# ReactiveBayes/RxInfer.jl

Measured on AMD Instinct MI355X. Metric: node-message-updates/sec (d=4 LGSSM, T=100k, BP sweep with Bethe free energy), higher is better.
Workload: dtype f64; 1 GPU; LGSSM d=4 dy=4 T=100000, 1024 independent chains per GPU (BASELINE config 2), 1 BP sweep + Bethe free energy per step; chain c drawn from numpy default_rng(42+c); chains_per_gpu=1024, T=100000, segments=128, segment_len=782

## Files before the change

### rxinfer.jl_amd/csrc/launch_tables.hpp

```cpp
#pragma once
#include <hip/hip_runtime.h>

#include <cstdlib>

#include "lgssm_kernels.hpp"
#include "predict_kernels.hpp"
#include "noise_kernels.hpp"
#ifndef RXHIP_LAUNCH_LGSSM_ONLY
#include "dense_kernels.hpp"
#include "dense_tab_kernels.hpp"
#include "dense_mseg_kernels.hpp"
#include "dense_split_kernels.hpp"
#include "dense8_kernels.hpp"
#endif

#ifndef RXHIP_TAB_SAME_TOL
#define RXHIP_TAB_SAME_TOL 5e-15
#endif

namespace rxhip {

struct SweepArgs {
    bool rev;
    int bnd;
    bool write_cov;
    int y_ring;
    int waves;
};
struct LgssmVtbl {
    int d, dy;
    int cst_size, tab_size, agg_size;
    int oA, oP, oLOBS, oG, oQI, oC0, oM1, oV1, oHF;
    int tK, tU;
    int aPI, aC, aJ, aCI, aX, aJJ;
    int scan_size, sM1, sM2, sVB, sN1, sN2, sLB;
    int f0_size, fK, fU, fSI, pos_size, pPI, pJ, pC, fs_size, fsA1, fsA2, fsW, mt_row;
    void (*forward0)(const Params&, const double*, bool, bool, int, hipStream_t);
    void (*time_tables)(const TimeTabParams&, hipStream_t);
    void (*fe_seg)(const Params&, hipStream_t);
    int gt_row, se_size;
    void (*smooth_tables)(const SmoothTabParams&, const double*, hipStream_t);
    void (*backward_sh)(const Params&, const double*, const double* gtab, const double* segend, const SweepArgs&, hipStream_t);
    void (*boundary_scan_tab)(const Params&, const double*, bool, hipStream_t);
    void (*seg_aggregate)(const Params&, const double*, bool, hipStream_t);
    int ex_size;
    void (*seg_elements)(const Params&, hipStream_t);
    void (*boundary_scan)(const Params&, const double*, bool, bool, hipStream_t);
    void (*forward)(const Params&, const double*, bool, bool, hipStream_t);
    void (*backward)(const Params&, const double*, bool, hipStream_t);
    void (*forecast)(const PredictParams&, hipStream_t);
    void (*predict)(const PredictParams&, hipStream_t);
    void (*joint)(const PredictParams&, hipStream_t);
    void (*stream_step)(const StreamParams&, hipStream_t);
    void (*small_sweep)(const Params&, const double*, bool, hipStream_t);
    int noise_prior_size;
    void (*noise_reset)(const NoiseParams&, hipStream_t);
    void (*noise_update)(const NoiseParams&, hipStream_t);
};
void lgssm_vtbls_d1(LgssmVtbl* out);
void lgssm_vtbls_d2(LgssmVtbl* out);
void lgssm_vtbls_d3(LgssmVtbl* out);
void lgssm_vtbls_d4(LgssmVtbl* out);

inline unsigned nblk(long long n, int b) { return (unsigned)((n + b - 1) / b); }

inline const char* hook_env(const char* name) {
    const char* on = std::getenv("RXHIP_TEST_HOOKS");
    return (on && on[0] == '1' && on[1] == 0) ? std::getenv(name) : nullptr;
}

#ifndef RXHIP_LAUNCH_LGSSM_ONLY
constexpr int FE_RESID_MAX_PASSES = 8;
struct DenseVtbl {
    int nt;
    hipError_t (*prepare)();
    void (*prepare_bnd)(const DenseParams&, hipStream_t);
    void (*seg_aggregate)(const DenseParams&, hipStream_t);
    void (*boundary_scan)(const DenseParams&, bool fe, hipStream_t);
    void (*forward)(const DenseParams&, bool fe, hipStream_t);
    void (*forward_info)(const DenseParams&, bool fe, hipStream_t, long long chains);
    void (*backward_info)(const DenseParams&, bool fe, hipStream_t, long long chains);
    void (*fe_resid)(const DenseParams&, hipStream_t, int passes);
    hipError_t (*tab_prepare)();
    hipError_t (*tab_build)(const TabParams&, hipStream_t);
    void (*tab_consts)(const TabParams&, unsigned models, size_t lds, hipStream_t);
    hipError_t (*mseg_prepare)();
    void (*mseg_sweep)(const MsegParams&, const DenseParams&, bool fe, bool filter, hipStream_t);
    void (*mseg_filter_out)(const MsegParams&, const DenseParams&, hipStream_t);
    hipError_t (*split_prepare)();
    void (*split_forward)(const SplitParams&, dim3 grid, hipStream_t);
    void (*split_backward)(const SplitParams&, dim3 grid, hipStream_t);
    void (*cross_from_records)(const DenseParams&, double* cross, dim3 grid, hipStream_t);
};
const DenseVtbl* dense_vtbl_nt1();
const DenseVtbl* dense_vtbl_nt2();
const DenseVtbl* dense_vtbl_nt3();
const DenseVtbl* dense_vtbl_nt4();
#endif

}
```

### rxinfer.jl_amd/csrc/lgssm_kernels.hpp

```cpp
#pragma once
#include <hip/hip_runtime.h>
#include <stdint.h>

namespace rxhip {

constexpr int ST_NOT_POSDEF = 1;
constexpr int ST_NONFINITE = 2;
__device__ __forceinline__ void lds_barrier() {
    __builtin_amdgcn_fence(__ATOMIC_RELEASE, "workgroup", "local");
    __builtin_amdgcn_s_barrier();
    __builtin_amdgcn_fence(__ATOMIC_ACQUIRE, "workgroup", "local");
}
__device__ __forceinline__ bool is_finite(double x) { return (__double2hiint(x) & 0x7ff00000) != 0x7ff00000; }

#ifndef RXHIP_NT_STORES
#define RXHIP_NT_STORES 0
#endif
typedef double rx_d2v __attribute__((ext_vector_type(2)));
__device__ __forceinline__ void stream_store(double2* p, double a, double b) {
#if RXHIP_NT_STORES
    rx_d2v v = {a, b};
    __builtin_nontemporal_store(v, reinterpret_cast<rx_d2v*>(p));
#else
    *p = make_double2(a, b);
#endif
}

__device__ __forceinline__ void lds_put(double2& dst, const rx_d2v v) { dst = make_double2(v.x, v.y); }
template <class T>
__device__ __forceinline__ void lds_put(T& dst, const T& v) { dst = v; }
template <int NPIECES, int W, class T = rx_d2v>
struct LdsStream {
    static constexpr int TPB = 64 * W;
    static constexpr int PPL = (NPIECES + TPB - 1) / TPB;
    const int tid;
    T tr[PPL];
    __device__ __forceinline__ explicit LdsStream(const int tid_) : tid(tid_) {}
    template <class Piece>
    __device__ __forceinline__ void fetch(Piece&& piece) {
#pragma unroll
        for (int k = 0; k < PPL; ++k) piece(k * TPB + tid, tr[k]);
    }
    template <class B>
    __device__ __forceinline__ void stash(B* buf) const {
#pragma unroll
        for (int k = 0; k < PPL; ++k) {
            const int idx = k * TPB + tid;
            if ((k + 1) * TPB <= NPIECES || idx < NPIECES) lds_put(buf[idx], tr[k]);
        }
    }
    static __device__ __forceinline__ void publish() {
        if constexpr (W == 1) {
            __builtin_amdgcn_fence(__ATOMIC_RELEASE, "wavefront");
            __builtin_amdgcn_wave_barrier();
        } else {
            __builtin_amdgcn_fence(__ATOMIC_RELEASE, "workgroup", "local");
            __builtin_amdgcn_s_barrier();
            __builtin_amdgcn_fence(__ATOMIC_ACQUIRE, "workgroup", "local");
        }
    }
    template <class B>
    __device__ __forceinline__ void flip(B* buf, const bool store = true) {
        __builtin_amdgcn_fence(__ATOMIC_ACQUIRE, "wavefront");
        __builtin_amdgcn_wave_barrier();
        if (store) stash(buf);
        publish();
    }
};

template <int D>
struct Dim {
    static constexpr int NS = D * (D + 1) / 2;
    static constexpr int NP = D + NS;
    static constexpr int NP2 = (NP + 1) / 2;
};

__host__ __device__ constexpr int sidx(int i, int j) { return i >= j ? i * (i + 1) / 2 + j : j * (j + 1) / 2 + i; }

template <int D>
struct Sym {
    double v[D * (D + 1) / 2];
    __device__ __forceinline__ double& operator()(int i, int j) { return v[sidx(i, j)]; }
    __device__ __forceinline__ const double& operator()(int i, int j) const { return v[sidx(i, j)]; }
};

// ... 1141 lines not shown
    }
    if (live) f0_epilogue<D, FE>(p, seg, chain, m, eta, q0);
}

template <int D, int DY, bool FE, int W>
__global__ void __launch_bounds__(64 * W) k_forward0_ck(Params p, const CstArg<CstLayout<D, DY>::SIZE> cb) {
    using FL = F0Layout<D, DY>;
    using FS = F0Stage<D, DY>;
    constexpr int MT = TimeTab<D>::MT;
    constexpr int U = FS::U, NPF = FS::NPF, NPC = FS::NPC;
    __shared__ double2 tbuf[2][NPC];
    const int wv = W > 1 ? __builtin_amdgcn_readfirstlane((int)(threadIdx.x >> 6)) : 0;
    const int lane = W > 1 ? (int)(threadIdx.x & 63) : (int)threadIdx.x;
    const long long g0 = ((long long)blockIdx.x * W + wv) * 64;
    const long long seg = g0 / p.n_chains;
    const long long chain = g0 - seg * p.n_chains + lane;
    const long long len = seg_len(p, seg);
    const CPtr c{cb.v};
    const long long t0 = seg * p.L + 1;
    const int lg = p.ck_log2;
    const long long kmask = (1LL << lg) - 1;
    const long long f_last = p.L * (FL::SIZE / 2) - 1;
    const long long m_last = p.T * (MT / 2) - 1;
    const rx_d2v* f2 = reinterpret_cast<const rx_d2v*>(p.ftab);
    const rx_d2v* m2 = reinterpret_cast<const rx_d2v*>(p.mtab);

    double m[D], eta[D], q0 = 0.0;
#pragma unroll
    for (int i = 0; i < D; ++i) m[i] = eta[i] = 0.0;
    if (len > 0) {
        LdsStream<NPC, W> ts(threadIdx.x);
        ts.fetch([](const int, rx_d2v& v) { v = rx_d2v{0.0, 0.0}; });
        auto has_ck = [&](long long i0) { return ((i0 + U) >> lg) != (i0 >> lg) || (i0 < len && len <= i0 + U); };
        auto chunk = [&](long long i0) {
            return [&, i0, ck = has_ck(i0)](int idx, rx_d2v& v) {
                idx = idx < NPC ? idx : NPC - 1;
                if (idx < NPF) {
                    const long long gi = i0 * (FL::SIZE / 2) + idx;
                    v = f2[gi < f_last ? gi : f_last];
                } else if (ck) {
                    const long long gi = (t0 + i0) * (MT / 2) + (idx - NPF);
                    v = m2[gi < m_last ? gi : m_last];
                }
            };
        };
        ts.fetch(chunk(0));
        ts.stash(tbuf[0]);
        ts.publish();

        double yb[U][DY], yn[U][DY];
        auto y_index = [&](long long i) { return t0 + (i < len ? i : len - 1); };
#pragma unroll
        for (int u = 0; u < U; ++u) load_y<DY>(p.y, y_index(u), p.n_chains, chain, yn[u]);
        auto step = [&](const int u, const long long i, const int b) __attribute__((always_inline)) {
            const double* tb = reinterpret_cast<const double*>(&tbuf[b][0]) + u * FL::SIZE;
            const double* mt = reinterpret_cast<const double*>(&tbuf[b][NPF]) + u * MT;
            f0_step<D, DY, FE>(c, tb, yb[u], m, eta, q0);
            if (((i + 1) & kmask) != 0 && i + 1 != len) return;
            f0_store_z<D>(p, 1 + seg * p.nck + (i >> lg), chain, m, eta, mt);
        };
        int b = 0;
        long long i0 = 0;
        for (; i0 + U <= len; i0 += U, b ^= 1) {
            ts.fetch(chunk(i0 + U));
#pragma unroll
            for (int u = 0; u < U; ++u) {
#pragma unroll
                for (int k = 0; k < DY; ++k) yb[u][k] = yn[u][k];
                load_y<DY>(p.y, y_index(i0 + U + u), p.n_chains, chain, yn[u]);
            }
#pragma unroll
            for (int u = 0; u < U; ++u) step(u, i0 + u, b);
            ts.flip(tbuf[b ^ 1]);
        }
#pragma unroll
        for (int u = 0; u < U; ++u)
#pragma unroll
            for (int k = 0; k < DY; ++k) yb[u][k] = yn[u][k];
#pragma unroll
        for (int u = 0; u < U - 1; ++u)
            if (i0 + u < len) step(u, i0 + u, b);
    }
    f0_epilogue<D, FE>(p, seg, chain, m, eta, q0);
}

struct TimeTabParams {
    long long T, L;
    const double* pos;
    const double* scan;
    double* mtab;
    double* ntab;
    double* vtab;
    int* status;
};
template <int D>
__global__ void __launch_bounds__(64) k_time_tables(TimeTabParams q) {
    using PL = PosLayout<D>;
    using SL = ScanLayout<D>;
    constexpr int NS = Dim<D>::NS;
    constexpr int MT = TimeTab<D>::MT;
    const long long t = (long long)blockIdx.x * blockDim.x + threadIdx.x;
    if (t >= q.T) return;
    if (t == 0) {
#pragma unroll
        for (int k = 0; k < NS; ++k) q.vtab[k] = q.scan[SL::VB + k];
#pragma unroll
        for (int k = 0; k < MT; ++k) q.mtab[k] = q.ntab[k] = 0.0;
        return;
    }
    const long long s = (t - 1) / q.L, i = t - s * q.L;
    const double* ps = q.pos + (i - 1) * PL::SIZE;
    const double* sc = q.scan + s * SL::SIZE;
    Sym<D> Vs, Vi, T1, W;
    double det;
    bool ok = true;
#pragma unroll
    for (int k = 0; k < NS; ++k) Vs.v[k] = sc[SL::VB + k];
    ok = spd_inv<D>(Vs, Vi, det) && ok;
#pragma unroll
    for (int k = 0; k < NS; ++k) T1.v[k] = Vi.v[k] + ps[PL::J + k];
    ok = spd_inv<D>(T1, W, det) && ok;
    double M[D][D], N[D][D];
#pragma unroll
    for (int a = 0; a < D; ++a)
#pragma unroll
        for (int b = 0; b < D; ++b) {
            double acc = 0.0;
#pragma unroll
            for (int k = 0; k < D; ++k) acc += ps[PL::PI + a * D + k] * W(k, b);
            M[a][b] = acc;
        }
#pragma unroll
    for (int a = 0; a < D; ++a)
#pragma unroll
        for (int b = 0; b < D; ++b) {
            double acc = 0.0;
#pragma unroll
            for (int k = 0; k < D; ++k) acc += M[a][k] * Vi(k, b);
            N[a][b] = acc;
        }
    double* mo = q.mtab + t * MT;
    double* no = q.ntab + t * MT;
#pragma unroll
    for (int a = 0; a < D; ++a)
#pragma unroll
        for (int b = 0; b < D; ++b) {
            mo[a * D + b] = M[a][b];
            no[a * D + b] = N[a][b];
        }
    if (D * D < MT) mo[MT - 1] = no[MT - 1] = 0.0;
    double* vo = q.vtab + t * NS;
#pragma unroll
    for (int a = 0; a < D; ++a)
#pragma unroll
        for (int b = 0; b <= a; ++b) {
            double acc = ps[PL::C + sidx(a, b)];
#pragma unroll
            for (int k = 0; k < D; ++k) acc += M[a][k] * ps[PL::PI + b * D + k];
            vo[sidx(a, b)] = acc;
        }
    if (!ok) atomicOr(q.status, ST_NOT_POSDEF);
}

template <int D>
__global__ void __launch_bounds__(64) k_fe_seg(Params p) {
    using FS = FeSegLayout<D>;
// ... 2106 lines not shown
```

### rxinfer.jl_amd/csrc/lgssm_plan.hpp

```cpp
#pragma once
#include <algorithm>
#include <cmath>
#include <cstdlib>
#include <cstring>
#include <string>

namespace rxhip {
namespace plan {

#define RXHIP_SCHEDULE_HOOKS(X)                                                                                                        \
    X(int, one_pass, -1)                                                                          \
    X(bool, one_segment, false)                                                                                  \
    X(bool, backward_lanes, false)                                                                            \
    X(bool, mean_records, false)                                                                              \
    X(int, mean_checkpoint, 0)                    \
    X(Text, mean_checkpoint_text, Text{})                                                   \
    X(bool, boundary_kernel, false)                                                                        \
    X(bool, small_sweep_off, false)                                                                            \
    X(bool, elem_full, false)                                                                                      \
    X(bool, noise_moments_pass, false)                                                                    \
    X(bool, no_pack, false)                                                                                          \
    X(int, dense_split, -1)                                      \
    X(bool, host_tables, false)                                                                                  \
    X(bool, gseq, false)                                                                                                \
    X(bool, stepm_gseq, false)                                                                                    \
    X(bool, filter_gseq, false)                                                                                  \
    X(bool, joints_gseq, false)                                                                                  \
    X(int, mseg_scan, 0)                                                 \
    X(bool, mseg_one_level, false)                                                                            \
    X(int, mseg_group, 0)                                                                          \
    X(unsigned long long, mseg_max_bytes, ~0ULL)                                         \
    X(bool, wave8_off, false)                                                                                        \
    X(bool, no_frozen, false)                                                                                      \
    X(bool, cov_every_sweep, false)                                                                        \
    X(int, y_ring, 0)                                      \
    X(int, sweep_waves, 0)

struct Text { char s[16] = {0}; };

struct ScheduleHooks {
#define X(type, field, dflt) type field = dflt;
    RXHIP_SCHEDULE_HOOKS(X)
#undef X
    template <class Get>
    static ScheduleHooks read(Get get) {
        ScheduleHooks h;
        auto set = [&](const char* n) { return get(n) != nullptr; };
        auto is0 = [&](const char* n) { const char* v = get(n); return v && std::atoi(v) == 0; };
        auto not0 = [&](const char* n) { const char* v = get(n); return v && std::atoi(v) != 0; };
        auto tri = [&](const char* n) { const char* v = get(n); return v ? (std::atoi(v) != 0 ? 1 : 0) : -1; };
        auto num = [&](const char* n) { const char* v = get(n); return v ? std::atoi(v) : 0; };
        h.one_pass = tri("RXHIP_ONE_PASS");
        h.one_segment = set("RXHIP_ONE_SEGMENT");
        h.backward_lanes = set("RXHIP_BACKWARD_LANES");
        h.mean_records = not0("RXHIP_MEAN_RECORDS");
        if (const char* v = get("RXHIP_MEAN_CHECKPOINT")) {
            h.mean_checkpoint = std::atoi(v);
            if (h.mean_checkpoint == 0) h.mean_checkpoint = -1;
            std::strncpy(h.mean_checkpoint_text.s, v, sizeof h.mean_checkpoint_text.s - 1);
        }
        h.boundary_kernel = not0("RXHIP_BOUNDARY_KERNEL");
        h.small_sweep_off = is0("RXHIP_SMALL_SWEEP");
        h.elem_full = set("RXHIP_ELEM_FULL");
        h.noise_moments_pass = set("RXHIP_NOISE_MOMENTS_PASS");
        h.no_pack = set("RXHIP_NO_PACK");
        h.dense_split = tri("RXHIP_DENSE_SPLIT");
        h.host_tables = set("RXHIP_HOST_TABLES");
        h.gseq = set("RXHIP_GSEQ");
        h.stepm_gseq = set("RXHIP_STEPM_GSEQ");
        h.filter_gseq = set("RXHIP_FILTER_GSEQ");
        h.joints_gseq = set("RXHIP_JOINTS_GSEQ");
        if (const char* v = get("RXHIP_MSEG_SCAN")) h.mseg_scan = !std::strcmp(v, "sequential") ? 1 : !std::strcmp(v, "log") ? 2 : 0;
        h.mseg_one_level = set("RXHIP_MSEG_ONE_LEVEL");
        h.mseg_group = num("RXHIP_MSEG_GROUP");
        if (const char* v = get("RXHIP_MSEG_MAX_BYTES")) h.mseg_max_bytes = std::strtoull(v, nullptr, 10);
        h.wave8_off = is0("RXHIP_WAVE8");
        h.no_frozen = set("RXHIP_NO_FROZEN");
        h.cov_every_sweep = not0("RXHIP_COV_EVERY_SWEEP");
        if (const char* v = get("RXHIP_Y_RING")) h.y_ring = !std::strcmp(v, "1") ? 1 : -1;
        if (const char* v = get("RXHIP_SWEEP_WAVES")) h.sweep_waves = !std::strcmp(v, "1") ? 1 : !std::strcmp(v, "2") ? 2 : !std::strcmp(v, "4") ? 4 : -1;
        return h;
    }
    void append_key(std::string& key) const {
#define X(type, field, dflt) key.append(reinterpret_cast<const char*>(&field), sizeof field);
        RXHIP_SCHEDULE_HOOKS(X)
#undef X
    }
};

struct Shape {
    int d = 0, dy = 0;
    long long T = 0, n_chains = 0;
    int n_models = 1;
    long long segments = 0;
    bool dense = false, allow_missing = false, step_model = false, chain_model = false;
};

struct Flags {
    bool sequential = false, uniform = true, gseq = false, masked = false;
    int dpad = 0, nt = 0;
    int pack = 1;
    long long wg_chains = 0;
    int dyk = 0;
};
inline Flags static_flags(const Shape& s, const ScheduleHooks& hooks) {
    Flags f;
    f.dpad = s.dense ? (s.d + 15) / 16 * 16 : s.d;
    f.nt = f.dpad / 16;
    f.uniform = (s.n_models == 1);
    if (s.allow_missing) {
        if (s.dense) f.gseq = true;
        f.masked = true;
        f.sequential = true;
        f.uniform = false;
    }
    if (s.step_model) {
        if (s.dense) f.gseq = true;
        f.sequential = true;
        f.uniform = false;
    }
    if (!s.dense && !f.uniform) f.sequential = true;
    f.pack = (s.dense && !f.gseq && s.d <= 8 && s.dy <= 32 && s.n_chains % 2 == 0 && s.n_models == 1 && !hooks.no_pack) ? 2 : 1;
    f.wg_chains = s.n_chains / f.pack;
    f.dyk = s.dy * f.pack;
    return f;
}

inline bool split_wanted(long long wg_chains, const ScheduleHooks& hooks) { return hooks.dense_split >= 0 ? hooks.dense_split != 0 : wg_chains >= 4; }

struct Segmentation {
    int S = 0;
    long long L = 1, Llast = 1;
    bool small_short = false;
};
inline Segmentation segmentation(const Shape& s, const Flags& f, const ScheduleHooks& hooks) {
    Segmentation g;
    const bool dense = s.dense;
    const bool dense_frozen = dense && f.nt >= 3 && f.uniform && !f.masked && !s.step_model && !f.gseq;
    const int dense_wg_per_cu = !dense ? 0 : f.nt == 1 ? 48 : f.nt == 2 ? 8 : dense_frozen ? 4 : 2;
    const long long steps = s.T - 1;
    if (steps <= 0) {
        g.S = 0;
        g.L = 1;
        g.Llast = 1;
        return g;
    }
    long long S_target = (f.sequential && hooks.one_segment) ? 1 : s.segments > 0 ? s.segments
                         : dense ? (256 * dense_wg_per_cu + f.wg_chains - 1) / f.wg_chains
                                 : (131072 + s.n_chains - 1) / s.n_chains;
    if (s.segments <= 0 && !dense) {
        const long long s_lat = (long long)std::ceil(std::sqrt(3.3 * (double)steps));
        if (S_target > s_lat) S_target = s_lat;
        const long long cap = s.n_chains <= 16 ? 256 / s.n_chains : 0;
        if (cap >= 1 && S_target > cap && (steps + cap - 1) / cap <= 32) S_target = cap;
        if (cap >= 1 && (steps + cap - 1) / cap <= 32 && f.uniform && !f.masked && !s.step_model && !hooks.small_sweep_off) {
            S_target = std::min<long long>(cap, std::max<long long>(1, steps / 3));
            g.small_short = true;
        }
    }
    const bool split_eligible = dense && !f.gseq && s.n_models == 1 && split_wanted(f.wg_chains, hooks);
    if (split_eligible && s.segments <= 0) S_target = std::max(S_target, std::min<long long>(128, (steps + 31) / 32));
    if (S_target < 1) S_target = 1;
    long long L = (steps + S_target - 1) / S_target;
// ... 29 lines not shown
```

### rxinfer.jl_amd/csrc/rxhip.hip

```cpp
#include "../../include/rxhip.h"

#include <hip/hip_runtime.h>

#include <algorithm>
#include <cmath>
#include <mutex>
#include <set>
#include <cstdarg>
#include <cstdio>
#include <cstring>
#include <cstdlib>
#include <string>
#include <vector>

#include "launch_tables.hpp"
#include "gseq_kernels.hpp"
#include "drift_kernels.hpp"
#include "generic_kernels.hpp"
#include "engine.hpp"
#include "graph_lowering.hpp"
#include "model_envelope.hpp"

using namespace rxhip;
using plan::ScheduleHooks;
// ... 1972 lines not shown
        ap.plain(&e->d_vstab, sizeof(double) * T * Du * Du);
        ap.plain(&e->d_fe_const, sizeof(double) * 2 * Sg);
    }
    if ((st = arena_commit(e, ap))) return st;
    tr.mark("dense: work buffers");
    return RXHIP_OK;
}
static rxhip_status lanes_time_tables(rxhip_engine* e, bool rev_cand, int ck_forced) {
    const LgssmVtbl* vt = e->vt;
    TimeTabParams q{};
    q.T = e->T; q.L = e->L; q.pos = e->d_pos; q.scan = e->d_scan; q.mtab = e->d_mtab; q.ntab = e->d_ntab; q.vtab = e->d_vtab;
    q.status = e->d_status;
    HIPCHK(e, hipEventCreate(&e->ev_tab0));
    HIPCHK(e, hipEventCreate(&e->ev_tab1));
    HIPCHK(e, hipEventRecord(e->ev_tab0, e->stream));
    vt->time_tables(q, e->stream);
    if (e->d_gtab) {
        SmoothTabParams sq{};
        sq.T = e->T; sq.L = e->L; sq.S = e->S; sq.vtab = e->d_vtab; sq.ntab = e->d_ntab; sq.scan = e->d_scan;
        sq.gtab = e->d_gtab; sq.segend = e->d_segend; sq.blk = e->d_sblk; sq.status = e->d_status;
        sq.rev = rev_cand ? 1 : 0; sq.amp = e->d_amp; sq.ainv = e->d_ainv; sq.ckfail = e->d_ckfail;
        vt->smooth_tables(sq, e->h_cst0.data(), e->stream);
        if (rev_cand) {
            int ckfail = 0;
            HIPCHK(e, hipMemcpyAsync(&ckfail, e->d_ckfail, sizeof(int), hipMemcpyDeviceToHost, e->stream));
            HIPCHK(e, hipStreamSynchronize(e->stream));
            e->ck_log2 = 0;
            if (ck_forced) {
                while ((1 << e->ck_log2) < ck_forced) ++e->ck_log2;
            } else {
                for (int k = 2; k >= 0 && !e->ck_log2; --k)
                    if (!((ckfail >> k) & 1)) e->ck_log2 = 3 + k;
            }
            if (!e->ck_log2) {
                sq.rev = 0;
                vt->smooth_tables(sq, e->h_cst0.data(), e->stream);
            }
        }
    }
    HIPCHK(e, hipEventRecord(e->ev_tab1, e->stream));
    HIPCHK(e, hipGetLastError());
    return RXHIP_OK;
}
static rxhip_status create_lanes(rxhip_engine* e, const rxhip_lgssm_desc* ds) {
    const LgssmVtbl* vt = e->vt;
    const size_t NP = (size_t)e->d + (size_t)e->d * (e->d + 1) / 2;
    const size_t NP2 = (NP + 1) / 2;
    const size_t Ltab = e->sequential ? 0 : (size_t)e->L;
    std::vector<double> cst((size_t)e->n_models * vt->cst_size), tab((size_t)e->n_models * Ltab * vt->tab_size + 1),
        agg((size_t)e->n_models * 2 * vt->agg_size), scan;
    FusedTables ft;
    const bool want_fused = plan::want_fused(e->uniform, e->S, e->n_chains, e->T, e->hooks);
    StageTrace tr(e->stage_ms);
    for (int m = 0; m < e->n_models; ++m) {
        rxhip_status st = build_model_tables(e, m, ds, cst.data() + (size_t)m * vt->cst_size,
                                             tab.data() + (size_t)m * Ltab * vt->tab_size,
                                             agg.data() + (size_t)m * 2 * vt->agg_size, e->uniform ? &scan : nullptr,
                                             want_fused ? &ft : nullptr);
        if (st) return st;
    }
    e->fused = want_fused && !scan.empty();
    e->fe_const = ft.fe_const;
    e->h_cst0.assign(cst.begin(), cst.begin() + vt->cst_size);
    tr.mark("lanes: host tables", STAGE_TABLES_HOST);
    const size_t C = (size_t)e->n_chains, T = (size_t)e->T, Sg = (size_t)(e->S > 0 ? e->S : 1);
    ArenaPlan ap;
    ap.upload(&e->d_cst, cst.data(), sizeof(double) * cst.size());
    ap.upload(&e->d_tab, tab.data(), sizeof(double) * tab.size());
    ap.upload(&e->d_agg, agg.data(), sizeof(double) * agg.size());
    if (ds->chain_model && !e->uniform) ap.upload(&e->d_chain_model, ds->chain_model, sizeof(int) * C);
    if (ds->step_model) ap.upload(&e->d_step_model, ds->step_model, sizeof(int) * (size_t)(e->T + e->H));
    if (!e->h_mu.empty()) {
        ap.upload(&e->d_mu, e->h_mu.data(), sizeof(double) * e->h_mu.size());
        ap.upload(&e->d_nu, e->h_nu.data(), sizeof(double) * e->h_nu.size());
        ap.upload(&e->d_cx, e->h_cx.data(), sizeof(double) * e->h_cx.size());
        ap.upload(&e->d_cy_raw, e->h_cy.data(), sizeof(double) * e->h_cy.size());
    }
    if (e->uniform && !scan.empty()) ap.upload(&e->d_scan, scan.data(), sizeof(double) * scan.size());
    const int ck_forced = e->hooks.mean_checkpoint;
    if (ck_forced && (ck_forced < 1 || ck_forced > 32 || (ck_forced & (ck_forced - 1))))
        return fail(e, RXHIP_ERR_BADARG, "RXHIP_MEAN_CHECKPOINT=%s: a power of two from 1 to 32", e->hooks.mean_checkpoint_text.s);
    if (e->hooks.y_ring != 0 && e->hooks.y_ring != 1)
        return fail(e, RXHIP_ERR_BADARG, "RXHIP_Y_RING: 1 (the depth-1 y ring of the reverse-filter sweep) or unset (depth %d)", Y_RING_SHIPPED);
    const int waves_forced = e->hooks.sweep_waves;
    if (waves_forced < 0)
        return fail(e, RXHIP_ERR_BADARG, "RXHIP_SWEEP_WAVES: 1, 2 or 4 (wavefronts per workgroup of the reverse-filter sweep kernels) or unset");
    if (waves_forced > 1 && !plan::sweep_waves_divide(e->n_chains, waves_forced))
        return fail(e, RXHIP_ERR_BADARG, "RXHIP_SWEEP_WAVES=%d: a workgroup of %d waves takes %d chains of one segment, which does not divide the batch of %lld",
                    waves_forced, waves_forced, 64 * waves_forced, (long long)e->n_chains);
    e->sweep_waves_fwd = plan::sweep_waves(e->n_chains, plan::SWEEP_WAVES_FORWARD, waves_forced);
    e->sweep_waves_bwd = plan::sweep_waves(e->n_chains, plan::SWEEP_WAVES_BACKWARD, waves_forced);
    const bool rev_cand = plan::rev_cand(e->fused, e->n_chains, e->d, e->dy, e->T, e->hooks);
    if (e->fused) {
        ap.upload(&e->d_ftab, ft.ftab.data(), sizeof(double) * ft.ftab.size());
        ap.upload(&e->d_pos, ft.pos.data(), sizeof(double) * ft.pos.size());
        ap.upload(&e->d_fseg, ft.fseg.data(), sizeof(double) * ft.fseg.size());
        ap.plain(&e->d_mtab, sizeof(double) * T * vt->mt_row);
        ap.plain(&e->d_ntab, sizeof(double) * T * vt->mt_row);
        if (plan::gtab_tables(e->n_chains, e->hooks)) {
            ap.plain(&e->d_gtab, sizeof(double) * T * vt->gt_row);
            ap.plain(&e->d_segend, sizeof(double) * Sg * vt->se_size);
            ap.plain(&e->d_sblk, sizeof(double) * Sg * (size_t)smooth_blocks_per_segment(e->L) * 3 * e->d * e->d);
        }
        if (rev_cand) {
            ap.plain(&e->d_amp, sizeof(double) * T);
            ap.zeroed(&e->d_ainv, sizeof(double) * e->d * e->d);
            ap.zeroed(&e->d_ckfail, sizeof(int));
        }
    }
    ap.zeroed_last(&e->d_status, sizeof(int));
    ap.zeroed(&e->d_fe_part, sizeof(double) * (Sg + 2) * C);
    e->fe_total_cap = 16;
    ap.zeroed(&e->d_fe_total, sizeof(double) * e->fe_total_cap);
    ap.plain(&e->d_fe_blocks, sizeof(double) * ((C + 63) / 64));
    if (e->uniform) {
        const size_t MP2 = ((size_t)e->d + 1) / 2;
        if (!rev_cand) ap.plain(&e->d_filt, sizeof(double) * T * MP2 * 2 * (((C + 63) / 64) * 64));
        ap.plain(&e->d_vtab, sizeof(double) * T * ((size_t)e->d * (e->d + 1) / 2));
    } else
        ap.plain(&e->d_filt, sizeof(double) * T * NP2 * 2 * (((C + 63) / 64) * 64));
    ap.plain_first(&e->d_mean, sizeof(double) * (size_t)e->Tout() * C * e->d);
    ap.plain_first(&e->d_cov, sizeof(double) * (size_t)e->Tout() * C * e->d * e->d);
    ap.plain_first(&e->d_fe_chain, sizeof(double) * C);
    ap.plain(&e->d_elem, sizeof(double) * Sg * 2 * e->d * C);
    if (e->sequential && e->S > 1) ap.plain(&e->d_elemx, sizeof(double) * Sg * vt->ex_size * C);
    ap.plain(&e->d_fstart, sizeof(double) * Sg * NP * C);
    ap.plain(&e->d_beta, sizeof(double) * (Sg + 1) * NP * C);
    if (sizeof(double) * T * C * e->dy <= ((size_t)64 << 20)) {
        ap.plain(&e->d_y, sizeof(double) * T * C * e->dy);
        e->own_y = true;
    }
    if (rxhip_status st = arena_commit(e, ap)) return st;
    tr.mark("lanes: arena", -1);
    if (e->fused) {
        if (rxhip_status st = lanes_time_tables(e, rev_cand, ck_forced)) return st;
        tr.mark("lanes: device tables (enqueued)", STAGE_TABLES_DEVICE);
    }
    if (rev_cand) {
        const size_t MP2 = ((size_t)e->d + 1) / 2;
        if (e->ck_log2) e->nck = (e->L + (1LL << e->ck_log2) - 1) >> e->ck_log2;
        const size_t slots = e->ck_log2 ? 1 + Sg * (size_t)e->nck : T;
        HIPCHK(e, hipMalloc(&e->d_filt, sizeof(double) * slots * MP2 * 2 * (((C + 63) / 64) * 64)));
    }
    return RXHIP_OK;
}

rxhip_status rxhip_lgssm_create(const rxhip_lgssm_desc* ds, rxhip_engine** out) {
    if (!out) return RXHIP_ERR_BADARG;
    *out = nullptr;
    const LgssmVtbl* vt = nullptr;
    bool dense = false;
    if (rxhip_status st = validate_desc(ds, &vt, &dense)) return st;
    if (dense && conditioning_guard().load())
        if (rxhip_status st = check_envelope(ds)) return st;
    const ScheduleHooks hooks = ScheduleHooks::read(hook_env);
    std::string pkey;
    if (engine_pool_key(ds, hooks, pkey))
        if (rxhip_engine* hit = engine_pool_take(pkey)) {
            *out = hit;
            return RXHIP_OK;
        }
    int ndev = 0;
    if (hipGetDeviceCount(&ndev) != hipSuccess || ndev <= 0) return RXHIP_ERR_NO_DEVICE;

    rxhip_engine* e = new rxhip_engine();
    *out = e;
// ... 479 lines not shown
    return RXHIP_OK;
}

static rxhip_status run_mseg(rxhip_engine* e, const RunPlan& pl) {
    if (rxhip_status st = mseg_run(e, pl.fe, pl.filter)) return st;
    e->records_hold_gains = !pl.filter && !e->m_wave8_last;
    return RXHIP_OK;
}
static rxhip_status run_gseq(rxhip_engine* e, const RunPlan& pl) {
    rxhip_status st;
    const bool fe = pl.fe, filter = pl.filter;
    GseqParams gq{};
    gq.T = e->T; gq.n_chains = e->n_chains; gq.d = e->d; gq.dy = e->dy; gq.ptt = e->ptt; gq.fe = fe ? 1 : 0; gq.y = e->d_y;
    gq.mean = e->d_mean; gq.cov = e->d_cov; gq.user = e->d_user; gq.prior = e->d_prior; gq.chain_model = e->d_chain_model;
    gq.step_model = e->d_step_model; gq.fe_part = e->d_fe_part; gq.status = e->d_status;
    const size_t lds = gseq_lds_bytes(e->d, e->dy);
    if ((st = prof_begin(e, RXHIP_K_FORWARD))) return st;
    hipLaunchKernelGGL(k_gseq_forward, dim3((unsigned)e->n_chains), dim3(256), lds, e->stream, gq);
    if ((st = prof_end(e))) return st;
    if (!filter && e->T > 1) {
        if ((st = prof_begin(e, RXHIP_K_BACKWARD))) return st;
        hipLaunchKernelGGL(k_gseq_backward, dim3((unsigned)e->n_chains), dim3(256), lds, e->stream, gq);
        if ((st = prof_end(e))) return st;
    }
    return RXHIP_OK;
}
static rxhip_status run_dense(rxhip_engine* e, const RunPlan& pl, const DenseParams& dp, bool was_cov_current, bool write_cov) {
    rxhip_status st;
    const bool fe = pl.fe, info = pl.info;
    if (pl.segments) {
        if ((st = prof_begin(e, RXHIP_K_SEG_AGGREGATE))) return st;
        DENSE_DISPATCH(e->nt, seg_aggregate(dp, e->stream));
        if ((st = prof_end(e))) return st;
    }
    if ((st = prof_begin(e, RXHIP_K_BOUNDARY_SCAN))) return st;
    DENSE_DISPATCH(e->nt, boundary_scan(dp, fe && !info, e->stream));
    if ((st = prof_end(e))) return st;
    if (pl.family == RunFamily::DenseSplit) {
        SplitParams sq{};
        sq.p = dp; sq.D = e->dpad; sq.rec = dense_rec(e->nt); sq.dtab = e->d_dtab; sq.vlast = e->d_vlast; sq.vstab = e->d_vstab;
        sq.fe_const = e->d_fe_const;
        if (!e->split_ready) {
            DenseParams mp = dp;
            mp.vlast = e->d_vlast;
            mp.full_records = 1;
            DENSE_DISPATCH(e->nt, forward_info(mp, true, e->stream, 1));
            DENSE_DISPATCH(e->nt, backward_info(mp, true, e->stream, 1));
            hipLaunchKernelGGL(kd_split_tables, dim3((unsigned)e->T), dim3(256), 0, e->stream, sq);
            hipLaunchKernelGGL(kd_split_save, dim3(256), dim3(256), 0, e->stream, sq, (long long)e->n_chains);
            e->split_ready = true;
        }
        if ((st = prof_begin(e, RXHIP_K_FORWARD))) return st;
        const long long per_wg = 4 * (64 / e->dpad);
        const dim3 lds_grid((unsigned)((e->wg_chains + per_wg - 1) / per_wg), (unsigned)e->S);
        dense_vt(e->nt)->split_forward(sq, lds_grid, e->stream);
        if ((st = prof_end(e))) return st;
        if ((st = prof_begin(e, RXHIP_K_BACKWARD))) return st;
        dense_vt(e->nt)->split_backward(sq, lds_grid, e->stream);
        const bool lazy = e->cov_mode == 1 && e->H == 0;
        if (lazy && was_cov_current) e->cov_current = true;
        else if (lazy) e->cov_pending = true;
        const bool store = !lazy && write_cov;
        hipLaunchKernelGGL(kd_split_broadcast, dim3(store ? 2048 : 64), dim3(256), 0, e->stream, sq, (long long)e->n_chains, fe ? 1 : 0, store ? 1 : 0);
        if ((st = prof_end(e))) return st;
    } else if (pl.segments) {
        if ((st = prof_begin(e, RXHIP_K_FORWARD))) return st;
        if (info) { DENSE_DISPATCH(e->nt, forward_info(dp, fe, e->stream, -1)); }
        else { DENSE_DISPATCH(e->nt, forward(dp, fe, e->stream)); }
        if ((st = prof_end(e))) return st;
        if (info) {
            if ((st = prof_begin(e, RXHIP_K_BACKWARD))) return st;
            DENSE_DISPATCH(e->nt, backward_info(dp, fe, e->stream, -1));
            e->records_hold_gains = e->pack == 1;
            if ((st = prof_end(e))) return st;
        }
    }
    return RXHIP_OK;
}
static rxhip_status run_lanes(rxhip_engine* e, const RunPlan& pl, const Params& p, bool write_cov) {
    rxhip_status st;
    const bool fe = pl.fe, fused = pl.family == RunFamily::OnePass, bnd_in_sweep = pl.bnd_in_sweep;
    if (fused) {
        if ((st = prof_begin(e, RXHIP_K_FORWARD))) return st;
        e->vt->forward0(p, e->h_cst0.data(), fe, e->ck_log2 > 0, e->sweep_waves_fwd, e->stream);
        if ((st = prof_end(e))) return st;
    } else if (pl.family == RunFamily::SmallSweep) {
        e->vt->small_sweep(p, e->h_cst0.data(), fe, e->stream);
        return RXHIP_OK;
    } else if (pl.family == RunFamily::FourPhase) {
        if ((st = prof_begin(e, RXHIP_K_SEG_AGGREGATE))) return st;
        e->vt->seg_aggregate(p, e->h_cst0.data(), e->uniform, e->stream);
        if ((st = prof_end(e))) return st;
    } else if (pl.elements_pass) {
        if ((st = prof_begin(e, RXHIP_K_SEG_AGGREGATE))) return st;
        e->vt->seg_elements(p, e->stream);
        if ((st = prof_end(e))) return st;
    }
    if (!bnd_in_sweep) {
        if ((st = prof_begin(e, RXHIP_K_BOUNDARY_SCAN))) return st;
        if (pl.scan_tab) e->vt->boundary_scan_tab(p, e->h_cst0.data(), fe, e->stream);
        else e->vt->boundary_scan(p, e->h_cst0.data(), e->uniform, fe, e->stream);
        if ((st = prof_end(e))) return st;
    }
    if (pl.segments) {
        if (!fused) {
            if ((st = prof_begin(e, RXHIP_K_FORWARD))) return st;
            e->vt->forward(p, e->h_cst0.data(), e->uniform, fe, e->stream);
            if ((st = prof_end(e))) return st;
        } else if (fe && !bnd_in_sweep)
            e->vt->fe_seg(p, e->stream);
        if (!pl.filter) {
            if ((st = prof_begin(e, RXHIP_K_BACKWARD))) return st;
            if (pl.backward_sh) {
                SweepArgs a;
                a.rev = e->ck_log2 > 0;
                a.bnd = bnd_in_sweep ? (fe ? 2 : 1) : 0;
                a.write_cov = write_cov;
                a.y_ring = e->hooks.y_ring == 1 ? 1 : Y_RING_SHIPPED;
                a.waves = e->sweep_waves_bwd;
                e->vt->backward_sh(p, e->h_cst0.data(), e->d_gtab, e->d_segend, a, e->stream);
            } else e->vt->backward(p, e->h_cst0.data(), e->uniform, e->stream);
            if ((st = prof_end(e))) return st;
        }
        if (fe && bnd_in_sweep) e->vt->fe_seg(p, e->stream);
    }
    return RXHIP_OK;
}
static rxhip_status run_tail(rxhip_engine* e, const RunPlan& pl, const Params& p, const DenseParams& dp, NoiseParams& np, int it) {
    rxhip_status st;
    if (e->noise) {
        np.iteration = it;
        e->vt->noise_update(np, e->stream);
    }
    if (pl.fe && pl.family != RunFamily::SmallSweep) {
        if ((st = prof_begin(e, RXHIP_K_FE_REDUCE))) return st;
        const int nb = (int)((e->n_chains + 63) / 64);
        Params pr = p;
        pr.S = pl.fe_slots;
        pr.fe_part = pl.fe_part;
        if (pl.info && (pl.family == RunFamily::Dense || pl.family == RunFamily::DenseSplit)) launch_fe_resid(dp, e->stream);
        if (e->n_chains <= 16) {
            hipLaunchKernelGGL(k_fe_few, dim3(1), dim3(256), 0, e->stream, pr);
        } else {
            hipLaunchKernelGGL(k_fe_chain, dim3(nb), dim3(256), 0, e->stream, pr, e->d_fe_blocks);
            hipLaunchKernelGGL(k_fe_total, dim3(1), dim3(256), 0, e->stream, p, (const double*)e->d_fe_blocks, nb);
        }
        if ((st = prof_end(e))) return st;
    }
    if (e->d_mu) {
        hipLaunchKernelGGL(k_shift_rows, dim3(2048), dim3(256), 0, e->stream, e->d_mean, (const double*)e->d_mu, e->T, e->n_chains, e->d, 1.0, e->off_chain ? 1 : 0);
    }
    if (e->H > 0 && e->dense) {
        GenericParams gp{};
        gp.T = e->T; gp.H = e->H; gp.n_chains = e->n_chains; gp.d = e->d; gp.dy = e->dy; gp.mean = e->d_mean; gp.cov = e->d_cov;
        gp.user = e->d_user; gp.cx = e->d_cx; gp.off_chain = e->off_chain ? 1 : 0; gp.chain_model = e->d_chain_model; gp.step_model = e->d_step_model; gp.status = e->d_status;
        hipLaunchKernelGGL(k_forecast_generic, dim3((unsigned)e->n_chains), dim3(256), generic_forecast_lds(e->d), e->stream, gp);
    }
    if (e->H > 0 && !e->dense) {
        PredictParams pp{};
        pp.T = e->T; pp.H = e->H; pp.n_chains = e->n_chains; pp.mean = e->d_mean; pp.cov = e->d_cov; pp.cst = e->d_cst;
        pp.chain_model = e->d_chain_model; pp.step_model = e->d_step_model; pp.status = e->d_status; pp.cx = e->d_cx; pp.off_chain = e->off_chain ? 1 : 0;
        e->vt->forecast(pp, e->stream);
    }
    return RXHIP_OK;
}

static rxhip_status run_impl(rxhip_engine* e, int32_t iterations, int32_t want_fe, bool filter) {
// ... 564 lines not shown
```

### rxinfer.jl_amd/csrc/tu_lgssm.hip

```cpp
#include <cstring>
#include <type_traits>

#define RXHIP_LAUNCH_LGSSM_ONLY
#include "launch_tables.hpp"

#ifndef RXHIP_TU_D
#error "compile with -DRXHIP_TU_D=1..4"
#endif

namespace rxhip {
namespace {

template <class F>
void pick(bool b, F&& f) {
    if (b) f(std::true_type{});
    else f(std::false_type{});
}
template <class F>
void pick_waves(int w, F&& f) {
    if (w == 4) f(std::integral_constant<int, 4>{});
    else if (w == 2) f(std::integral_constant<int, 2>{});
    else f(std::integral_constant<int, 1>{});
}

template <int D, int DY>
struct Launch {
    using CL = CstLayout<D, DY>;
    static CstArg<CL::SIZE> carg(const double* hc) {
        CstArg<CL::SIZE> a;
        std::memcpy(a.v, hc, sizeof(double) * CL::SIZE);
        return a;
    }
    static void seg_aggregate(const Params& p, const double* hc, bool uni, hipStream_t s) {
        const long long total = p.n_chains * (long long)p.S;
        if (uni) hipLaunchKernelGGL((k_seg_aggregate<D, DY, true>), dim3(nblk(total, 64)), dim3(64), 0, s, p, carg(hc));
    }
    static void seg_elements(const Params& p, hipStream_t s) {
        if (!p.masked && !p.step_model && !p.elem_full && p.L >= 384) {
            hipLaunchKernelGGL((k_seg_elements<D, DY, true>), dim3(nblk(p.n_chains * (long long)p.S, 64)), dim3(64), 0, s, p);
            hipLaunchKernelGGL((k_seg_elements_tail<D, DY>), dim3(nblk(p.n_chains * (long long)p.S, 64)), dim3(64), 0, s, p);
        } else hipLaunchKernelGGL((k_seg_elements<D, DY, false>), dim3(nblk(p.n_chains * (long long)p.S, 64)), dim3(64), 0, s, p);
    }
    static void boundary_scan(const Params& p, const double* hc, bool uni, bool fe, hipStream_t s) {
        dim3 grid(nblk(p.n_chains, 64), p.filter ? 1 : 2);
        pick(fe, [&](auto FE) {
            if (uni) hipLaunchKernelGGL((k_boundary_scan<D, DY, true, FE()>), grid, dim3(64), 0, s, p, carg(hc));
            else if (!p.masked && !p.step_model && !p.elem_full)
                hipLaunchKernelGGL((k_boundary_scan<D, DY, false, FE(), true>), grid, dim3(64), 0, s, p, CstArg<1>{});
            else hipLaunchKernelGGL((k_boundary_scan<D, DY, false, FE()>), grid, dim3(64), 0, s, p, CstArg<1>{});
        });
    }
    static void boundary_scan_tab(const Params& p, const double* hc, bool fe, hipStream_t s) {
        dim3 grid(nblk(p.n_chains, 64), p.filter ? 1 : 2);
        pick(fe, [&](auto FE) { hipLaunchKernelGGL((k_boundary_scan_tab<D, DY, FE()>), grid, dim3(64), 0, s, p, carg(hc)); });
    }
    template <bool FILT>
    static void forward_t(const Params& p, const double* hc, bool uni, bool fe, hipStream_t s) {
        const long long total = p.n_chains * (long long)p.S;
        dim3 grid(nblk(total, 64));
        pick(fe, [&](auto FE) {
            if (uni) hipLaunchKernelGGL((k_forward<D, DY, true, FE(), FILT>), grid, dim3(64), 0, s, p, carg(hc));
            else if (!FILT && p.tinv_records) hipLaunchKernelGGL((k_forward_tinv<D, DY, FE()>), grid, dim3(64), 0, s, p);
            else hipLaunchKernelGGL((k_forward<D, DY, false, FE(), FILT>), grid, dim3(64), 0, s, p, CstArg<1>{});
        });
    }
    static void forward(const Params& p, const double* hc, bool uni, bool fe, hipStream_t s) {
        pick(p.filter != 0, [&](auto FILT) { forward_t<FILT()>(p, hc, uni, fe, s); });
    }
    static void backward(const Params& p, const double* hc, bool uni, hipStream_t s) {
        const long long total = p.n_chains * (long long)p.S;
        dim3 grid(nblk(total, 64));
        if (uni && p.ntab) hipLaunchKernelGGL((k_backward<D, DY, true, true>), grid, dim3(64), 0, s, p, carg(hc));
        else if (uni) hipLaunchKernelGGL((k_backward<D, DY, true>), grid, dim3(64), 0, s, p, carg(hc));
        else if (p.noise_part && p.tinv_records) hipLaunchKernelGGL((k_backward_noise<D, DY, true>), grid, dim3(64), 0, s, p);
        else if (p.noise_part) hipLaunchKernelGGL((k_backward_noise<D, DY>), grid, dim3(64), 0, s, p);
        else if (p.tinv_records) hipLaunchKernelGGL((k_backward_tinv<D, DY>), grid, dim3(64), 0, s, p);
        else hipLaunchKernelGGL((k_backward<D, DY, false>), grid, dim3(64), 0, s, p, CstArg<1>{});
    }
    static void forward0(const Params& p, const double* hc, bool fe, bool ck, int waves, hipStream_t s) {
        const long long total = p.n_chains * (long long)p.S;
        pick(fe, [&](auto FE) {
            if (ck)
                pick_waves(waves, [&](auto W) {
                    hipLaunchKernelGGL((k_forward0_ck<D, DY, FE(), W()>), dim3((unsigned)(p.n_chains / (64 * W()) * p.S)), dim3(64 * W()), 0, s, p, carg(hc));
                });
            else hipLaunchKernelGGL((k_forward0<D, DY, FE()>), dim3(nblk(total, 64)), dim3(64), 0, s, p, carg(hc));
        });
    }
    static void time_tables(const TimeTabParams& q, hipStream_t s) {
        hipLaunchKernelGGL((k_time_tables<D>), dim3(nblk(q.T, 64)), dim3(64), 0, s, q);
    }
    static void fe_seg(const Params& p, hipStream_t s) {
        hipLaunchKernelGGL((k_fe_seg<D>), dim3(nblk(p.n_chains * (long long)p.S, 64)), dim3(64), 0, s, p);
    }
    static void smooth_tables(const SmoothTabParams& q, const double* hc, hipStream_t s) {
        const long long nblocks = (long long)q.S * smooth_blocks_per_segment(q.L);
        if (q.T > 1) hipLaunchKernelGGL((k_smooth_tab_steps<D, DY>), dim3(nblk(q.T - 1, 64)), dim3(64), 0, s, q, carg(hc));
        hipLaunchKernelGGL((k_smooth_tab_compose<D>), dim3(nblk(nblocks, 64)), dim3(64), 0, s, q);
        hipLaunchKernelGGL((k_smooth_tab_chain<D>), dim3(nblk(q.S, 64)), dim3(64), 0, s, q);
        hipLaunchKernelGGL((k_smooth_tab_apply<D>), dim3(nblk(nblocks, 64)), dim3(64), 0, s, q);
    }
    static void backward_sh(const Params& p, const double* hc, const double* gtab, const double* segend, const SweepArgs& a, hipStream_t s) {
        const int write_cov = a.write_cov ? 1 : 0;
        if (!a.rev) {
            hipLaunchKernelGGL((k_backward_sh<D>), dim3((unsigned)(p.n_chains / 64 * p.S)), dim3(64), 0, s, p, gtab, segend, write_cov);
            return;
        }
        pick_waves(a.waves, [&](auto W) {
            pick(a.y_ring == 1, [&](auto R1) {
                constexpr int R = R1() ? 1 : Y_RING_SHIPPED;
                hipLaunchKernelGGL((k_backward_sh_rev<D, DY, R, W()>), dim3((unsigned)(p.n_chains / (64 * W()) * p.S)), dim3(64 * W()), 0, s, p, gtab, segend,
                                   carg(hc), a.bnd, write_cov);
            });
        });
    }
    static void forecast(const PredictParams& p, hipStream_t s) {
        hipLaunchKernelGGL((k_forecast<D, DY>), dim3(nblk(p.n_chains, 64)), dim3(64), 0, s, p);
    }
    static void predict(const PredictParams& p, hipStream_t s) {
        const long long total = (p.T + p.H) * p.n_chains;
        const long long nb = (total + 255) / 256;
        hipLaunchKernelGGL((k_predict<D, DY>), dim3((unsigned)(nb < 8192 ? nb : 8192)), dim3(256), 0, s, p);
    }
    static void joint(const PredictParams& p, hipStream_t s) {
        const long long nb = ((p.T - 1) * p.n_chains + 255) / 256;
        hipLaunchKernelGGL((k_joint<D, DY>), dim3((unsigned)(nb < 8192 ? (nb > 0 ? nb : 1) : 8192)), dim3(256), 0, s, p);
    }
    static void small_sweep(const Params& p, const double* hc, bool fe, hipStream_t s) {
        const size_t lds = sizeof(double) * (size_t)small_sweep_lds_doubles<D, DY>();
        const int par = p.S >= 24 ? 1 : 0;
        pick(fe, [&](auto FE) {
            pick(p.filter != 0, [&](auto FILT) {
                hipLaunchKernelGGL((k_small_sweep<D, DY, FE(), FILT()>), dim3(1), dim3(SMALL_SWEEP_THREADS), lds, s, p, carg(hc), par);
            });
        });
    }
    static void noise_reset(const NoiseParams& p, hipStream_t s) {
        hipLaunchKernelGGL((k_noise_reset<D, DY>), dim3(nblk(p.n_chains, 64)), dim3(64), 0, s, p);
    }
    static void noise_update(const NoiseParams& p, hipStream_t s) {
        if (!p.moments_in_sweep) hipLaunchKernelGGL((k_noise_moments<D, DY>), dim3(nblk(p.n_chains, 64), (unsigned)p.slices), dim3(64), 0, s, p);
        hipLaunchKernelGGL((k_noise_update<D, DY>), dim3(nblk(p.n_chains, 64)), dim3(64), 0, s, p);
    }
    static void stream_step(const StreamParams& p, hipStream_t s) {
        hipLaunchKernelGGL((k_stream_step<D, DY>), dim3(nblk(p.n_chains, 64)), dim3(64), 0, s, p);
    }
    static LgssmVtbl vtbl() {
        using TL = TabLayout<D, DY>;
        using AL = AggLayout<D>;
        LgssmVtbl v;
        v.d = D; v.dy = DY;
        v.cst_size = CL::SIZE; v.tab_size = TL::SIZE; v.agg_size = AL::SIZE;
        v.oA = CL::A; v.oP = CL::P; v.oLOBS = CL::LOBS; v.oG = CL::G; v.oQI = CL::QI; v.oC0 = CL::C0;
        v.oM1 = CL::M1; v.oV1 = CL::V1; v.oHF = CL::HF;
        v.tK = TL::K; v.tU = TL::U;
        v.aPI = AL::PI; v.aC = AL::C; v.aJ = AL::J; v.aCI = AL::CI; v.aX = AL::X; v.aJJ = AL::JJ;
        using SL = ScanLayout<D>;
        v.scan_size = SL::SIZE; v.sM1 = SL::M1; v.sM2 = SL::M2; v.sVB = SL::VB; v.sN1 = SL::N1; v.sN2 = SL::N2; v.sLB = SL::LB;
        using FL = F0Layout<D, DY>;
        using PL = PosLayout<D>;
        using FS = FeSegLayout<D>;
        v.f0_size = FL::SIZE; v.fK = FL::K; v.fU = FL::U; v.fSI = FL::SI;
        v.pos_size = PL::SIZE; v.pPI = PL::PI; v.pJ = PL::J; v.pC = PL::C;
// ... 39 lines not shown
```

Before: 294.6 billion rule-calls/s.

## Run one-pass forward filter step on matrix cores via f64 MFMA for d=4

Adds a forward-filter kernel for D=4, DY=4 that packs the per-step affine recurrence (A, H, gain, U, S^-1 blocks) into 16x16x4 f64 MFMA operands. Each wave processes four groups of 16 chains, and each time step becomes two or three matrix-core instructions instead of scalar VALU FMAs. It becomes the default for this config, with an env hook to fall back to the VALU kernel. The risk is wasted MFMA lanes from the padded operand layout, plus the added register pressure and prefetch ring on a latency-bound serial chain.

```diff
diff --git a/rxinfer.jl_amd/csrc/f0_pack.hpp b/rxinfer.jl_amd/csrc/f0_pack.hpp
--- /dev/null
+++ b/rxinfer.jl_amd/csrc/f0_pack.hpp
@@ -0,0 +1,37 @@
+#pragma once
+
+#if defined(__HIPCC__) || defined(__CUDACC__)
+#define RXHIP_F0_HD __host__ __device__
+#else
+#define RXHIP_F0_HD
+#endif
+
+namespace rxhip {
+namespace f0mx {
+
+RXHIP_F0_HD constexpr int lane_block(int lane) { return (lane & 15) >> 2; }
+RXHIP_F0_HD constexpr int lane_row(int lane) { return lane & 3; }
+RXHIP_F0_HD constexpr int lane_col(int lane) { return lane >> 4; }
+RXHIP_F0_HD constexpr int packed_sym(int i, int j) { return i >= j ? i * (i + 1) / 2 + j : j * (j + 1) / 2 + i; }
+
+RXHIP_F0_HD constexpr int x1_offset(int D, int DY, int oHF, int oA, int lane, bool& negate) {
+    const int r = lane_block(lane), a = lane_row(lane), k = lane_col(lane);
+    negate = r == 2;
+    if (r == 0 && a < D && k < D) return oA + a * D + k;
+    if (r == 2 && a < DY && k < D) return oHF + a * D + k;
+    return -1;
+}
+RXHIP_F0_HD constexpr int x2_offset(int D, int DY, int oK, int oU, int oSI, bool fe, int lane) {
+    const int r = lane_block(lane), a = lane_row(lane), k = lane_col(lane);
+    if (r == 0 && a < D && k < DY) return oK + a * DY + k;
+    if (r == 1 && a < D && k < DY) return oU + a * DY + k;
+    if (r == 3 && fe && a < DY && k < DY) return oSI + packed_sym(a, k);
+    return -1;
+}
+RXHIP_F0_HD constexpr int x3_offset(int D, int lane) {
+    const int r = lane_block(lane), a = lane_row(lane), k = lane_col(lane);
+    return (r == 0 && a < D && k < D) ? a * D + k : -1;
+}
+
+}
+}
diff --git a/rxinfer.jl_amd/csrc/launch_tables.hpp b/rxinfer.jl_amd/csrc/launch_tables.hpp
--- a/rxinfer.jl_amd/csrc/launch_tables.hpp
+++ b/rxinfer.jl_amd/csrc/launch_tables.hpp
@@ -35,7 +35,7 @@
     int aPI, aC, aJ, aCI, aX, aJJ;
     int scan_size, sM1, sM2, sVB, sN1, sN2, sLB;
     int f0_size, fK, fU, fSI, pos_size, pPI, pJ, pC, fs_size, fsA1, fsA2, fsW, mt_row;
-    void (*forward0)(const Params&, const double*, bool, bool, int, hipStream_t);
+    void (*forward0)(const Params&, const double*, bool fe, bool ck, int waves, bool valu, hipStream_t);
     void (*time_tables)(const TimeTabParams&, hipStream_t);
     void (*fe_seg)(const Params&, hipStream_t);
     int gt_row, se_size;
diff --git a/rxinfer.jl_amd/csrc/lgssm_kernels.hpp b/rxinfer.jl_amd/csrc/lgssm_kernels.hpp
--- a/rxinfer.jl_amd/csrc/lgssm_kernels.hpp
+++ b/rxinfer.jl_amd/csrc/lgssm_kernels.hpp
@@ -1,6 +1,8 @@
 #pragma once
 #include <hip/hip_runtime.h>
 #include <stdint.h>
+
+#include "f0_pack.hpp"
 
 namespace rxhip {
 
@@ -1308,6 +1310,164 @@
             if (i0 + u < len) step(u, i0 + u, b);
     }
     f0_epilogue<D, FE>(p, seg, chain, m, eta, q0);
+}
+
+typedef double rx_d4v __attribute__((ext_vector_type(4)));
+template <int D, int DY>
+struct F0Mx {
+    static constexpr bool ON = D == 4 && DY == 4;
+};
+template <int D, int DY, bool FE, bool CK>
+__global__ void __launch_bounds__(64, 2) k_forward0_mx(Params p) {
+    using CL = CstLayout<D, DY>;
+    using FL = F0Layout<D, DY>;
+    constexpr int MT = TimeTab<D>::MT, MP2 = DimM<D>::MP2;
+    constexpr int G = 4;
+    constexpr int R = CK ? 8 : 2;
+    constexpr int NM = CK ? 1 : G;
+    const int lane = threadIdx.x, j = lane & 15, q = lane >> 4;
+    const long long total = p.n_chains * (long long)p.S;
+    const long long g0 = (long long)blockIdx.x * 64;
+    auto uni = [](const long long v) {
+        return (long long)(((unsigned long long)(unsigned)__builtin_amdgcn_readfirstlane((int)(v >> 32)) << 32) | (unsigned)__builtin_amdgcn_readfirstlane((int)v));
+    };
+    long long seg[G], len[G], t0[G], chain[G];
+#pragma unroll
+    for (int g = 0; g < G; ++g) {
+        if (CK && g > 0) {
+            seg[g] = seg[0]; len[g] = len[0]; t0[g] = t0[0];
+            chain[g] = chain[0] + 16 * g;
+            continue;
+        }
+        const long long gg = g0 + 16 * g;
+        const bool live = gg < total;
+        seg[g] = live ? uni(gg / p.n_chains) : 0;
+        len[g] = live ? seg_len(p, seg[g]) : 0;
+        t0[g] = seg[g] * p.L + 1;
+        chain[g] = (live ? gg - seg[g] * p.n_chains : 0) + j;
+    }
+    const long long steps = CK ? len[0] : p.L;
+    const int lg = p.ck_log2;
+    const long long kmask = (1LL << lg) - 1;
+    auto stores_z = [&](const long long i) { return !CK || ((i + 1) & kmask) == 0 || i + 1 == len[0]; };
+
+    bool neg1;
+    const int o1 = f0mx::x1_offset(D, DY, CL::HF, CL::A, lane, neg1);
+    const int o2 = f0mx::x2_offset(D, DY, FL::K, FL::U, FL::SI, FE, lane);
+    const int o3 = f0mx::x3_offset(D, lane);
+    const bool has2 = o2 >= 0, has3 = o3 >= 0, hasy = q < DY;
+    double x1 = 0.0;
+    if (o1 >= 0) x1 = neg1 ? -p.cst[o1] : p.cst[o1];
+    const double* f_lane = p.ftab + (has2 ? o2 : 0);
+    const double* m_lane = p.mtab + (has3 ? o3 : 0);
+    const double* y_lane[G];
+    long long z_lane[G];
+#pragma unroll
+    for (int g = 0; g < G; ++g) {
+        y_lane[g] = p.y + chain[g] * DY + (hasy ? q : 0);
+        z_lane[g] = (((chain[g] >> 6) * MP2 + (q >> 1)) * 64 + (chain[g] & 63)) * 2 + (q & 1);
+    }
+    const long long y_row = p.n_chains * DY, z_slot = p.nb64 * MP2 * 128;
+
+    double yr[R][G], x2r[R], x3r[R][NM];
+#pragma unroll
+    for (int u = 0; u < R; ++u)
+#pragma unroll
+        for (int k = 0; k < NM; ++k) x3r[u][k] = 0.0;
+    auto fetch = [&](const int u, const long long i) __attribute__((always_inline)) {
+#pragma unroll
+        for (int g = 0; g < G; ++g) {
+            long long ii = i < len[g] ? i : len[g] - 1;
+            ii = ii > 0 ? ii : 0;
+            yr[u][g] = y_lane[g][(t0[g] + ii) * y_row];
+        }
+        x2r[u] = f_lane[(i < p.L ? i : p.L - 1) * FL::SIZE];
+        if (stores_z(i)) {
+#pragma unroll
+            for (int k = 0; k < NM; ++k) {
+                const long long t = t0[k] + i;
+                x3r[u][k] = m_lane[(t < p.T ? t : p.T - 1) * MT];
+            }
+        }
+    };
+
+    rx_d4v c[G], w[G], cz[NM];
+    double eta[G], q0[G];
+#pragma unroll
+    for (int k = 0; k < NM; ++k) {
+        cz[k] = (rx_d4v){0.0, 0.0, 0.0, 0.0};
+        asm volatile("" : "+v"(cz[k]));
+    }
+#pragma unroll
+    for (int g = 0; g < G; ++g) {
+        c[g] = w[g] = (rx_d4v){0.0, 0.0, 0.0, 0.0};
+        asm volatile("" : "+v"(c[g]));
+        eta[g] = q0[g] = 0.0;
+    }
+    auto finish = [&](const int g) __attribute__((always_inline)) {
+        if (q < D) {
+            double* o = p.elem + (seg[g] * 2 * D + q) * p.n_chains + chain[g];
+            o[0] = w[g][0];
+            o[D * p.n_chains] = eta[g];
+        }
+        if (FE) {
+            double s = __shfl(q0[g], j, 64);
+#pragma unroll
+            for (int k = 1; k < 4; ++k) s += __shfl(q0[g], 16 * k + j, 64);
+            if (q == 0) p.fe_part[(seg[g] + 1) * p.n_chains + chain[g]] = -0.5 * s;
+        }
+    };
+    auto step = [&](const int u, const long long i) __attribute__((always_inline)) {
+        const double x2 = has2 ? x2r[u] : 0.0;
+#pragma unroll
+        for (int g = 0; g < G; ++g) {
+            c[g][2] = (DY == 4 || hasy) ? yr[u][g] : 0.0;
+            w[g] = __builtin_amdgcn_mfma_f64_16x16x4f64(x1, w[g][0], c[g], 0, 0, 0);
+        }
+#pragma unroll
+        for (int g = 0; g < G; ++g) w[g] = __builtin_amdgcn_mfma_f64_16x16x4f64(x2, w[g][2], w[g], 0, 0, 0);
+#pragma unroll
+        for (int g = 0; g < G; ++g) {
+            eta[g] += w[g][1];
+            if (FE) {
+                q0[g] = __builtin_fma(w[g][3], w[g][2], q0[g]);
+                asm volatile("" : "+v"(q0[g]));
+            }
+        }
+        if (stores_z(i)) {
+#pragma unroll
+            for (int g = 0; g < G; ++g) {
+                rx_d4v& t = cz[CK ? 0 : g];
+                const double x3 = has3 ? x3r[u][CK ? 0 : g] : 0.0;
+                double mz = w[g][0];
+                asm volatile("" : "+v"(mz));
+                t[0] = mz;
+                t = __builtin_amdgcn_mfma_f64_16x16x4f64(x3, eta[g], t, 0, 0, 0);
+                const long long slot = CK ? 1 + seg[0] * p.nck + (i >> lg) : t0[g] + i;
+                if ((CK || i < len[g]) && q < 2 * MP2) p.filt[slot * z_slot + z_lane[g]] = t[0];
+            }
+        }
+        if (!CK) {
+#pragma unroll
+            for (int g = 0; g < G; ++g)
+                if (i + 1 == len[g]) finish(g);
+        }
+    };
+
+#pragma unroll
+    for (int u = 0; u < R; ++u) fetch(u, u);
+    for (long long i0 = 0; i0 < steps; i0 += R) {
+#pragma unroll
+        for (int u = 0; u < R; ++u) {
+            if (u > 0 && i0 + u >= steps) break;
+            step(u, i0 + u);
+            fetch(u, i0 + R + u);
+        }
+    }
+    if (CK) {
+#pragma unroll
+        for (int g = 0; g < G; ++g) finish(g);
+    }
 }
 
 struct TimeTabParams {
diff --git a/rxinfer.jl_amd/csrc/lgssm_plan.hpp b/rxinfer.jl_amd/csrc/lgssm_plan.hpp
--- a/rxinfer.jl_amd/csrc/lgssm_plan.hpp
+++ b/rxinfer.jl_amd/csrc/lgssm_plan.hpp
@@ -34,7 +34,8 @@
     X(bool, no_frozen, false)                                                                                      \
     X(bool, cov_every_sweep, false)                                                                        \
     X(int, y_ring, 0)                                      \
-    X(int, sweep_waves, 0)
+    X(int, sweep_waves, 0)                 \
+    X(int, f0_valu, 0)
 
 struct Text { char s[16] = {0}; };
 
@@ -79,6 +80,7 @@
         h.cov_every_sweep = not0("RXHIP_COV_EVERY_SWEEP");
         if (const char* v = get("RXHIP_Y_RING")) h.y_ring = !std::strcmp(v, "1") ? 1 : -1;
         if (const char* v = get("RXHIP_SWEEP_WAVES")) h.sweep_waves = !std::strcmp(v, "1") ? 1 : !std::strcmp(v, "2") ? 2 : !std::strcmp(v, "4") ? 4 : -1;
+        if (const char* v = get("RXHIP_F0_VALU")) h.f0_valu = !std::strcmp(v, "1") ? 1 : -1;
         return h;
     }
     void append_key(std::string& key) const {
diff --git a/rxinfer.jl_amd/csrc/rxhip.hip b/rxinfer.jl_amd/csrc/rxhip.hip
--- a/rxinfer.jl_amd/csrc/rxhip.hip
+++ b/rxinfer.jl_amd/csrc/rxhip.hip
@@ -2078,6 +2078,8 @@
         return fail(e, RXHIP_ERR_BADARG, "RXHIP_MEAN_CHECKPOINT=%s: a power of two from 1 to 32", e->hooks.mean_checkpoint_text.s);
     if (e->hooks.y_ring != 0 && e->hooks.y_ring != 1)
         return fail(e, RXHIP_ERR_BADARG, "RXHIP_Y_RING: 1 (the depth-1 y ring of the reverse-filter sweep) or unset (depth %d)", Y_RING_SHIPPED);
+    if (e->hooks.f0_valu != 0 && e->hooks.f0_valu != 1)
+        return fail(e, RXHIP_ERR_BADARG, "RXHIP_F0_VALU: 1 (the forward kernels of the one-pass schedule on the VALU step) or unset (the matrix-core step)");
     const int waves_forced = e->hooks.sweep_waves;
     if (waves_forced < 0)
         return fail(e, RXHIP_ERR_BADARG, "RXHIP_SWEEP_WAVES: 1, 2 or 4 (wavefronts per workgroup of the reverse-filter sweep kernels) or unset");
@@ -2723,7 +2725,7 @@
     const bool fe = pl.fe, fused = pl.family == RunFamily::OnePass, bnd_in_sweep = pl.bnd_in_sweep;
     if (fused) {
         if ((st = prof_begin(e, RXHIP_K_FORWARD))) return st;
-        e->vt->forward0(p, e->h_cst0.data(), fe, e->ck_log2 > 0, e->sweep_waves_fwd, e->stream);
+        e->vt->forward0(p, e->h_cst0.data(), fe, e->ck_log2 > 0, e->sweep_waves_fwd, e->hooks.f0_valu == 1, e->stream);
         if ((st = prof_end(e))) return st;
     } else if (pl.family == RunFamily::SmallSweep) {
         e->vt->small_sweep(p, e->h_cst0.data(), fe, e->stream);
diff --git a/rxinfer.jl_amd/csrc/tu_lgssm.hip b/rxinfer.jl_amd/csrc/tu_lgssm.hip
--- a/rxinfer.jl_amd/csrc/tu_lgssm.hip
+++ b/rxinfer.jl_amd/csrc/tu_lgssm.hip
@@ -77,8 +77,16 @@
         else if (p.tinv_records) hipLaunchKernelGGL((k_backward_tinv<D, DY>), grid, dim3(64), 0, s, p);
         else hipLaunchKernelGGL((k_backward<D, DY, false>), grid, dim3(64), 0, s, p, CstArg<1>{});
     }
-    static void forward0(const Params& p, const double* hc, bool fe, bool ck, int waves, hipStream_t s) {
-        const long long total = p.n_chains * (long long)p.S;
+    static void forward0(const Params& p, const double* hc, bool fe, bool ck, int waves, bool valu, hipStream_t s) {
+        const long long total = p.n_chains * (long long)p.S;
+        if constexpr (F0Mx<D, DY>::ON) {
+            if (!valu && p.n_chains % 16 == 0) {
+                pick(fe, [&](auto FE) {
+                    pick(ck, [&](auto CK) { hipLaunchKernelGGL((k_forward0_mx<D, DY, FE(), CK()>), dim3(nblk(total, 64)), dim3(64), 0, s, p); });
+                });
+                return;
+            }
+        }
         pick(fe, [&](auto FE) {
             if (ck)
                 pick_waves(waves, [&](auto W) {
```

Result: no change. 294.6 billion rule-calls/s (median of 3 runs) (+0.0%).
